# myscale/MyScaleDB

Hardware: NVIDIA H100
Metric: QPS @ recall@10>=0.95 (exact: recall 1.0), FLAT brute-force IP top-10, 10M x 768-d bf16, batch 1024 (higher is better)
Workload: dtype bf16

## Files before the change

### myscaledb_b200/csrc/gemm_common.cuh

```cuda
#pragma once
#include <cuda.h>

#include "common.cuh"
#include "kernels.h"

namespace b200 {
namespace gemm {


constexpr int BM = 128;
constexpr int BN = 256;
constexpr int HN = 128;
constexpr int BK = 64;
constexpr int UMMA_K = 16;
constexpr int EPI_THREADS = 128;
constexpr int NUM_THREADS = EPI_THREADS + 32;
constexpr int SMEM_ALIGN_SLACK = 1024;
constexpr int MAX_STAGES = 4;
constexpr int SMEM_LIMIT = kSmemOptinBytes;

constexpr int SCRATCH_BYTES = 32 * EPI_THREADS * 4;
constexpr int ACC_COLS = 64;
constexpr int ACC_LD = BM + 4;
constexpr int ACC_BYTES = ACC_COLS * ACC_LD * 4;

enum class Operand { BF16, TF32X3, B1 };

template <Operand OP>
struct Layout {
    static constexpr bool F32X3 = OP == Operand::TF32X3;
    static constexpr int KB = F32X3 ? 32 : OP == Operand::B1 ? 128 : 64;
    static constexpr int MMA_K = F32X3 ? 8 : OP == Operand::B1 ? 32 : 16;
    static constexpr int A_PLANE = BM * 128;
    static constexpr int B_PLANE = HN * 128;
    static constexpr int PLANES = F32X3 ? 2 : 1;
    static constexpr int STAGE_BYTES = PLANES * (A_PLANE + B_PLANE);
    static constexpr int TX_BYTES = STAGE_BYTES - (PLANES - 1) * B_PLANE;
    __host__ __device__ static constexpr int off_acc(int st) { return st * STAGE_BYTES; }
    __host__ __device__ static constexpr int off_side(int st) { return off_acc(st) + ACC_BYTES; }
    __host__ __device__ static constexpr int off_bar(int st) { return off_side(st) + 2 * BN * 4; }
    __host__ __device__ static constexpr int off_scratch(int st) { return off_bar(st) + 256; }
    __host__ __device__ static constexpr int off_list(int st) { return off_scratch(st) + SCRATCH_BYTES; }
};

__device__ __forceinline__ void mbar_init(uint64_t *bar, uint32_t count) {
    asm volatile("mbarrier.init.shared::cta.b64 [%0], %1;" ::"r"(smem_u32(bar)), "r"(count));
}
__device__ __forceinline__ void mbar_arrive_expect_tx(uint64_t *bar, uint32_t bytes) {
    asm volatile("mbarrier.arrive.expect_tx.shared::cta.b64 _, [%0], %1;" ::"r"(smem_u32(bar)), "r"(bytes) : "memory");
}
__device__ __forceinline__ void mbar_arrive(uint64_t *bar) {
    asm volatile("mbarrier.arrive.shared::cta.b64 _, [%0];" ::"r"(smem_u32(bar)) : "memory");
}
__device__ __forceinline__ bool mbar_try_wait(uint32_t addr, uint32_t parity) {
    uint32_t ok;
    asm volatile(
        "{\n\t"
        ".reg .pred p;\n\t"
        "mbarrier.try_wait.parity.shared::cta.b64 p, [%1], %2;\n\t"
        "selp.u32 %0, 1, 0, p;\n\t"
        "}\n"
        : "=r"(ok)
        : "r"(addr), "r"(parity)
        : "memory");
    return ok != 0;
}
__device__ __forceinline__ void mbar_wait(uint64_t *bar, uint32_t parity) {
    const uint32_t addr = smem_u32(bar);
    while (!mbar_try_wait(addr, parity)) {
    }
}

__device__ __forceinline__ void tma_load_2d(const CUtensorMap *map, uint64_t *bar, void *dst, int c0, int c1) {
    asm volatile(
        "cp.async.bulk.tensor.2d.shared::cluster.global.mbarrier::complete_tx::bytes [%0], [%1, {%3, %4}], [%2];" ::"r"(
            smem_u32(dst)),
        "l"(reinterpret_cast<uint64_t>(map)), "r"(smem_u32(bar)), "r"(c0), "r"(c1)
        : "memory");
}

__device__ __forceinline__ bool elect_one() {
    uint32_t pred;
    asm volatile(
        "{\n\t"
        ".reg .pred P;\n\t"
        "elect.sync _|P, 0xffffffff;\n\t"
        "selp.b32 %0, 1, 0, P;\n\t"
        "}\n"
        : "=r"(pred));
    return pred != 0;
}

__device__ __forceinline__ uint32_t bound_encode(float f) {
    const uint32_t b = __float_as_uint(f);
    return (b & 0x80000000u) ? ~b : (b | 0x80000000u);
}
__device__ __forceinline__ float bound_decode(uint32_t u) { return (u & 0x80000000u) ? __uint_as_float(u & 0x7fffffffu) : __uint_as_float(~u); }

__device__ __forceinline__ void wg_bar() { asm volatile("bar.sync 1, 128;" ::: "memory"); }

__device__ __forceinline__ uint64_t make_smem_desc(uint32_t smem_addr) {
    uint64_t d = 0;
    d |= (uint64_t)((smem_addr >> 4) & 0x3FFF);
    d |= (uint64_t)1 << 16;
    d |= (uint64_t)(1024 >> 4) << 32;
    d |= (uint64_t)1 << 62;
    return d;
}

__device__ __forceinline__ void wgmma_fence() { asm volatile("wgmma.fence.sync.aligned;" ::: "memory"); }
__device__ __forceinline__ void wgmma_commit() { asm volatile("wgmma.commit_group.sync.aligned;" ::: "memory"); }
template <int N>
__device__ __forceinline__ void wgmma_wait() { asm volatile("wgmma.wait_group.sync.aligned %0;" ::"n"(N) : "memory"); }

#define B200_ACC64_AS(C, v)                                                                                                     \
    C(v[0]), C(v[1]), C(v[2]), C(v[3]), C(v[4]), C(v[5]), C(v[6]), C(v[7]), C(v[8]), C(v[9]), C(v[10]), C(v[11]), C(v[12]),     \
        C(v[13]), C(v[14]), C(v[15]), C(v[16]), C(v[17]), C(v[18]), C(v[19]), C(v[20]), C(v[21]), C(v[22]), C(v[23]), C(v[24]), \
        C(v[25]), C(v[26]), C(v[27]), C(v[28]), C(v[29]), C(v[30]), C(v[31]), C(v[32]), C(v[33]), C(v[34]), C(v[35]), C(v[36]), \
        C(v[37]), C(v[38]), C(v[39]), C(v[40]), C(v[41]), C(v[42]), C(v[43]), C(v[44]), C(v[45]), C(v[46]), C(v[47]), C(v[48]), \
        C(v[49]), C(v[50]), C(v[51]), C(v[52]), C(v[53]), C(v[54]), C(v[55]), C(v[56]), C(v[57]), C(v[58]), C(v[59]), C(v[60]), \
        C(v[61]), C(v[62]), C(v[63])
#define B200_ACC64(v) B200_ACC64_AS("+f", v)
#define B200_ACC64_REGS                                                                                                         \
    "{%0, %1, %2, %3, %4, %5, %6, %7, %8, %9, %10, %11, %12, %13, %14, %15, %16, %17, %18, %19, %20, %21, %22, %23, %24, %25, " \
    "%26, %27, %28, %29, %30, %31, %32, %33, %34, %35, %36, %37, %38, %39, %40, %41, %42, %43, %44, %45, %46, %47, %48, %49, "   \
    "%50, %51, %52, %53, %54, %55, %56, %57, %58, %59, %60, %61, %62, %63}"

__device__ __forceinline__ void wgmma_bf16_n128(float (&d)[64], uint64_t adesc, uint64_t bdesc, uint32_t accum) {
    asm volatile(
        "{\n\t"
        ".reg .pred p;\n\t"
        "setp.ne.b32 p, %66, 0;\n\t"
        "wgmma.mma_async.sync.aligned.m64n128k16.f32.bf16.bf16 " B200_ACC64_REGS ", %64, %65, p, 1, 1, 0, 0;\n\t"
        "}\n"
        : B200_ACC64(d)
        : "l"(adesc), "l"(bdesc), "r"(accum));
}
__device__ __forceinline__ void wgmma_tf32_n128(float (&d)[64], uint64_t adesc, uint64_t bdesc, uint32_t accum) {
    asm volatile(
        "{\n\t"
        ".reg .pred p;\n\t"
        "setp.ne.b32 p, %66, 0;\n\t"
        "wgmma.mma_async.sync.aligned.m64n128k8.f32.tf32.tf32 " B200_ACC64_REGS ", %64, %65, p, 1, 1;\n\t"
        "}\n"
        : B200_ACC64(d)
        : "l"(adesc), "l"(bdesc), "r"(accum));
}
__device__ __forceinline__ void wgmma_b1_n128(int32_t (&d)[64], uint64_t adesc, uint64_t bdesc, uint32_t accum) {
    asm volatile(
        "{\n\t"
        ".reg .pred p;\n\t"
        "setp.ne.b32 p, %66, 0;\n\t"
        "wgmma.mma_async.sync.aligned.m64n128k256.s32.b1.b1.and.popc " B200_ACC64_REGS ", %64, %65, p;\n\t"
        "}\n"
        : B200_ACC64_AS("+r", d)
        : "l"(adesc), "l"(bdesc), "r"(accum));
}

template <int Q, typename T>
__device__ __forceinline__ void acc_store(float *acc, const T (&d0)[64], const T (&d1)[64]) {
    const int warp = (threadIdx.x >> 5) & 3, lane = threadIdx.x & 31;
    const int r = warp * 16 + (lane >> 2), c = 2 * (lane & 3);
#pragma unroll
    for (int j = 0; j < ACC_COLS / 8; j++) {
        const int i = Q * (ACC_COLS / 8) + j;
        float *col = acc + (8 * j + c) * ACC_LD + r;
        col[0] = (float)d0[4 * i];
        col[ACC_LD] = (float)d0[4 * i + 1];
        col[8] = (float)d0[4 * i + 2];
        col[ACC_LD + 8] = (float)d0[4 * i + 3];
        col[64] = (float)d1[4 * i];
        col[ACC_LD + 64] = (float)d1[4 * i + 1];
        col[72] = (float)d1[4 * i + 2];
        col[ACC_LD + 72] = (float)d1[4 * i + 3];
    }
}
__device__ __forceinline__ void acc_load32(const float *acc, int row, int c0, float (&v)[32]) {
    const float *p = acc + c0 * ACC_LD + row;
#pragma unroll
    for (int j = 0; j < 32; j++) v[j] = p[j * ACC_LD];
}

struct ThreadTopK {
    float *keys;
    uint32_t *ids;
    int k, n, worst;
    int tourn;
    float thr_key;
    uint32_t thr_id;
};

__device__ __forceinline__ void list_bind(ThreadTopK &t, float *keys_base, uint32_t *ids_base, int row, int k) {
    t.k = k;
    t.tourn = k >= list_tourn_min_k ? 1 : 0;
    t.keys = keys_base + row;
    t.ids = ids_base + row;
}

__device__ __forceinline__ void list_insert(ThreadTopK &t, float key, uint32_t id) {
    if (!better(key, id, t.thr_key, t.thr_id)) return;
    if (t.tourn) {
        const int G = list_tourn_group(t.k);
        const int ng = (t.k + G - 1) / G;
        if (t.n < t.k) {
            t.keys[t.n * EPI_THREADS] = key;
            t.ids[t.n * EPI_THREADS] = id;
            t.n++;
            if (t.n < t.k) return;
            for (int g = 0; g < ng; g++) {
                const int base = g * G, end = base + G < t.k ? base + G : t.k;
                float wk = t.keys[base * EPI_THREADS];
                uint32_t wi = t.ids[base * EPI_THREADS];
                for (int j = base + 1; j < end; j++) {
                    const float kj = t.keys[j * EPI_THREADS];
                    const uint32_t ij = t.ids[j * EPI_THREADS];
                    if (better(wk, wi, kj, ij)) {
                        wk = kj;
                        wi = ij;
                    }
                }
                t.keys[(t.k + g) * EPI_THREADS] = wk;
                t.ids[(t.k + g) * EPI_THREADS] = wi;
            }
        } else {
            const int g = t.worst;
            const int base = g * G, end = base + G < t.k ? base + G : t.k;
            float wk = 0.f;
            uint32_t wi = 0;
            int slot = -1;
            bool have = false;
            for (int j = base; j < end; j++) {
                float kj = t.keys[j * EPI_THREADS];
                uint32_t ij = t.ids[j * EPI_THREADS];
                if (slot < 0 && kj == t.thr_key && ij == t.thr_id) {
                    slot = j;
                    kj = key;
                    ij = id;
                }
                if (!have || better(wk, wi, kj, ij)) {
                    wk = kj;
                    wi = ij;
                    have = true;
                }
            }
            if (slot < 0) slot = base;
            t.keys[slot * EPI_THREADS] = key;
            t.ids[slot * EPI_THREADS] = id;
            t.keys[(t.k + g) * EPI_THREADS] = wk;
            t.ids[(t.k + g) * EPI_THREADS] = wi;
        }
        float wk = t.keys[t.k * EPI_THREADS];
        uint32_t wi = t.ids[t.k * EPI_THREADS];
        int wg = 0;
        for (int g = 1; g < ng; g++) {
            const float kg = t.keys[(t.k + g) * EPI_THREADS];
            const uint32_t ig = t.ids[(t.k + g) * EPI_THREADS];
            if (better(wk, wi, kg, ig)) {
                wk = kg;
                wi = ig;
                wg = g;
            }
        }
        t.worst = wg;
        t.thr_key = wk;
        t.thr_id = wi;
        return;
    }
    if (t.n < t.k) {
        t.keys[t.n * EPI_THREADS] = key;
        t.ids[t.n * EPI_THREADS] = id;
        t.n++;
        if (t.n < t.k) return;
    } else {
        t.keys[t.worst * EPI_THREADS] = key;
        t.ids[t.worst * EPI_THREADS] = id;
    }
    float wk = t.keys[0];
    uint32_t wi = t.ids[0];
    int wp = 0;
    for (int j = 1; j < t.k; j++) {
        const float kj = t.keys[j * EPI_THREADS];
        const uint32_t ij = t.ids[j * EPI_THREADS];
        if (better(wk, wi, kj, ij)) {
            wk = kj;
            wi = ij;
            wp = j;
        }
    }
    t.worst = wp;
    t.thr_key = wk;
    t.thr_id = wi;
}

static __device__ __noinline__ void list_publish(ThreadTopK &t, float *out_keys, uint32_t *out_ids) {
    for (int i = 1; i < t.n; i++) {
        const float ki = t.keys[i * EPI_THREADS];
        const uint32_t ii = t.ids[i * EPI_THREADS];
        int j = i;
        while (j > 0 && better(ki, ii, t.keys[(j - 1) * EPI_THREADS], t.ids[(j - 1) * EPI_THREADS])) {
            t.keys[j * EPI_THREADS] = t.keys[(j - 1) * EPI_THREADS];
            t.ids[j * EPI_THREADS] = t.ids[(j - 1) * EPI_THREADS];
            j--;
        }
        t.keys[j * EPI_THREADS] = ki;
        t.ids[j * EPI_THREADS] = ii;
    }
    for (int j = 0; j < t.k; j++) {
        out_keys[j] = j < t.n ? t.keys[j * EPI_THREADS] : FLT_MAX;
        out_ids[j] = j < t.n ? t.ids[j * EPI_THREADS] : kNoId;
    }
}

__device__ __forceinline__ void side_fma32(float (&v)[32], const float *scale, const float *bias) {
    const uint32_t sa = smem_u32(scale), ba = smem_u32(bias);
#pragma unroll
    for (int j = 0; j < 32; j += 4) {
        float s0, s1, s2, s3, b0, b1, b2, b3;
        asm volatile("ld.shared.v4.f32 {%0, %1, %2, %3}, [%4];" : "=f"(s0), "=f"(s1), "=f"(s2), "=f"(s3) : "r"(sa + j * 4));
        asm volatile("ld.shared.v4.f32 {%0, %1, %2, %3}, [%4];" : "=f"(b0), "=f"(b1), "=f"(b2), "=f"(b3) : "r"(ba + j * 4));
        v[j] = fmaf(v[j], s0, b0);
        v[j + 1] = fmaf(v[j + 1], s1, b1);
        v[j + 2] = fmaf(v[j + 2], s2, b2);
        v[j + 3] = fmaf(v[j + 3], s3, b3);
    }
}

__device__ __forceinline__ float jaccard_negkey(float v, int pq, float scale, float popc_y) {
    const bool live = scale != 0.f;
    const int x_and = (int)v, x_or = pq + (live ? (int)popc_y : 0) - x_and;
    const float key = x_or == 0 ? 0.f : (float)(x_or - x_and) / (float)x_or;
    return live ? -key : __int_as_float(0xff800000);
}

__device__ __forceinline__ void jaccard_keys32(float (&v)[32], int pq, const float *scale, const float *popc_y) {
    const uint32_t sa = smem_u32(scale), ba = smem_u32(popc_y);
#pragma unroll
    for (int j = 0; j < 32; j += 4) {
        float s[4], b[4];
        asm volatile("ld.shared.v4.f32 {%0, %1, %2, %3}, [%4];" : "=f"(s[0]), "=f"(s[1]), "=f"(s[2]), "=f"(s[3]) : "r"(sa + j * 4));
        asm volatile("ld.shared.v4.f32 {%0, %1, %2, %3}, [%4];" : "=f"(b[0]), "=f"(b[1]), "=f"(b[2]), "=f"(b[3]) : "r"(ba + j * 4));
#pragma unroll
        for (int i = 0; i < 4; i++) v[j + i] = jaccard_negkey(v[j + i], pq, s[i], b[i]);
    }
}

template <int LD = EPI_THREADS>
__device__ __forceinline__ void epilogue_chunk(ThreadTopK &list, float (&v)[32], bool use_side, const float *scale,
                                               const float *bias, uint32_t id0, bool tail, int64_t n, float *scratch,
                                               float ext_bound = FLT_MAX ) {
    const float thr = fminf(list.thr_key, ext_bound);
    bool mine;
    if (use_side) {
        side_fma32(v, scale, bias);
        float m0 = fminf(v[0], v[1]), m1 = fminf(v[2], v[3]), m2 = fminf(v[4], v[5]), m3 = fminf(v[6], v[7]);
#pragma unroll
        for (int j = 8; j < 32; j += 8) {
            m0 = fminf(m0, fminf(v[j], v[j + 1]));
            m1 = fminf(m1, fminf(v[j + 2], v[j + 3]));
            m2 = fminf(m2, fminf(v[j + 4], v[j + 5]));
            m3 = fminf(m3, fminf(v[j + 6], v[j + 7]));
        }
        mine = fminf(fminf(m0, m1), fminf(m2, m3)) <= thr;
    } else {
        float m0 = fmaxf(v[0], v[1]), m1 = fmaxf(v[2], v[3]), m2 = fmaxf(v[4], v[5]), m3 = fmaxf(v[6], v[7]);
#pragma unroll
        for (int j = 8; j < 32; j += 8) {
            m0 = fmaxf(m0, fmaxf(v[j], v[j + 1]));
            m1 = fmaxf(m1, fmaxf(v[j + 2], v[j + 3]));
            m2 = fmaxf(m2, fmaxf(v[j + 4], v[j + 5]));
            m3 = fmaxf(m3, fmaxf(v[j + 6], v[j + 7]));
        }
        mine = fmaxf(fmaxf(m0, m1), fmaxf(m2, m3)) >= -thr;
    }
    if (__any_sync(0xffffffffu, mine)) {
        uint32_t mask = 0;
#pragma unroll
        for (int j = 0; j < 32; j++) {
            const float key = use_side ? v[j] : -v[j];
            scratch[j * LD] = key;
            if (key <= thr) mask |= 1u << j;
        }
        if (tail && !use_side) {
            const int64_t left = n - (int64_t)id0;
            mask = left >= 32 ? mask : left <= 0 ? 0u : (mask & ((1u << left) - 1u));
        }
        while (__any_sync(0xffffffffu, mask != 0)) {
            if (mask) {
                const int j = __ffs(mask) - 1;
                mask &= mask - 1;
                list_insert(list, scratch[j * LD], id0 + (uint32_t)j);
            }
        }
    }
}

typedef CUresult (*EncodeTiledFn)(CUtensorMap *, CUtensorMapDataType, cuuint32_t, void *, const cuuint64_t *,
                                  const cuuint64_t *, const cuuint32_t *, const cuuint32_t *, CUtensorMapInterleave,
                                  CUtensorMapSwizzle, CUtensorMapL2promotion, CUtensorMapFloatOOBfill);

inline EncodeTiledFn get_encode_fn() {
    static EncodeTiledFn fn = nullptr;
    static bool tried = false;
    if (!tried) {
        tried = true;
        void *ptr = nullptr;
        cudaDriverEntryPointQueryResult qres;
        if (cudaGetDriverEntryPoint("cuTensorMapEncodeTiled", &ptr, cudaEnableDefault, &qres) == cudaSuccess &&
            qres == cudaDriverEntryPointSuccess)
            fn = reinterpret_cast<EncodeTiledFn>(ptr);
    }
    return fn;
}

inline bool encode_rows_map(CUtensorMap *map, const void *base, int64_t rows, int d_pad, int box_rows) {
    EncodeTiledFn fn = get_encode_fn();
    if (!fn) return false;
    const cuuint64_t dims[2] = {(cuuint64_t)d_pad, (cuuint64_t)rows};
    const cuuint64_t strides[1] = {(cuuint64_t)d_pad * 2};
    const cuuint32_t box[2] = {(cuuint32_t)BK, (cuuint32_t)box_rows};
    const cuuint32_t estr[2] = {1, 1};
    return fn(map, CU_TENSOR_MAP_DATA_TYPE_BFLOAT16, 2, const_cast<void *>(base), dims, strides, box, estr,
              CU_TENSOR_MAP_INTERLEAVE_NONE, CU_TENSOR_MAP_SWIZZLE_128B, CU_TENSOR_MAP_L2_PROMOTION_L2_256B,
              CU_TENSOR_MAP_FLOAT_OOB_FILL_NONE) == CUDA_SUCCESS;
}

inline bool encode_bytes_map(CUtensorMap *map, const void *base, int64_t rows, int row_bytes, int box_rows) {
    EncodeTiledFn fn = get_encode_fn();
    if (!fn) return false;
    const cuuint64_t dims[2] = {(cuuint64_t)row_bytes, (cuuint64_t)rows};
    const cuuint64_t strides[1] = {(cuuint64_t)row_bytes};
    const cuuint32_t box[2] = {128, (cuuint32_t)box_rows};
    const cuuint32_t estr[2] = {1, 1};
    return fn(map, CU_TENSOR_MAP_DATA_TYPE_UINT8, 2, const_cast<void *>(base), dims, strides, box, estr,
              CU_TENSOR_MAP_INTERLEAVE_NONE, CU_TENSOR_MAP_SWIZZLE_128B, CU_TENSOR_MAP_L2_PROMOTION_L2_256B,
              CU_TENSOR_MAP_FLOAT_OOB_FILL_NONE) == CUDA_SUCCESS;
}

}
}
```

### myscaledb_b200/csrc/ip_gemm_sm90.cu

```cuda
#include <cstdlib>
#include <type_traits>

#include "gemm_common.cuh"

namespace b200 {
namespace gemm {

template <Operand OP>
struct Op {
    using L = Layout<OP>;
    using Acc = typename std::conditional<OP == Operand::B1, int32_t, float>::type;
    static constexpr bool F32X3 = L::F32X3;
    static constexpr int KB = L::KB, MMA_K = L::MMA_K, A_PLANE = L::A_PLANE, B_PLANE = L::B_PLANE, PLANES = L::PLANES;
    static constexpr int WG = gemm_consumer_warpgroups(F32X3);
    static constexpr int THREADS = WG == 1 ? EPI_THREADS + 32 : 3 * EPI_THREADS;
    static constexpr int PRODUCER_REGS = 40, CONSUMER_REGS = 232;
    static constexpr int B_ROWS = WG * HN;
    static constexpr int PASSES = BN / B_ROWS;
    static constexpr int STAGE_BYTES = PLANES * (A_PLANE + WG * B_PLANE);
    static constexpr int TX_BYTES = PLANES * A_PLANE + WG * B_PLANE;
    static constexpr int STAGING_BYTES = 32 * 32 * 4;
    static constexpr int MAX_ST = F32X3 ? 2 : 3;
    static_assert(MAX_ST <= MAX_STAGES, "barrier arrays");
    __host__ __device__ static constexpr int off_staging(int st) { return st * STAGE_BYTES; }
    __host__ __device__ static constexpr int off_bar(int st) { return off_staging(st) + WG * 4 * STAGING_BYTES; }
    __host__ __device__ static constexpr int off_list(int st) { return off_bar(st) + 256; }
    static constexpr int list_bytes(int k_smem) { return k_smem * EPI_THREADS * 8; }
    static size_t smem_bytes(int st, int k_smem) { return (size_t)off_list(st) + (size_t)WG * list_bytes(k_smem) + SMEM_ALIGN_SLACK; }
    static bool lists_fit(int k_smem) { return smem_bytes(2, k_smem) <= (size_t)SMEM_LIMIT; }
    static int stages_for(int k_smem) {
        int st = MAX_ST;
        while (st > 2 && smem_bytes(st, k_smem) > (size_t)SMEM_LIMIT) st--;
        return st;
    }
};

template <int N>
__device__ __forceinline__ void setmaxnreg_inc() { asm volatile("setmaxnreg.inc.sync.aligned.u32 %0;" ::"n"(N)); }
template <int N>
__device__ __forceinline__ void setmaxnreg_dec() { asm volatile("setmaxnreg.dec.sync.aligned.u32 %0;" ::"n"(N)); }

__device__ __forceinline__ void wg_bar(int wg) { asm volatile("bar.sync %0, 128;" ::"r"(wg + 1) : "memory"); }

__device__ __forceinline__ int slot_row(int warp, int slot) { return (slot < 16 ? 0 : 48) + 16 * warp + slot; }

__device__ __forceinline__ float acc_f32(float x) { return x; }
__device__ __forceinline__ float acc_f32(int32_t x) { return __int_as_float(x); }
template <int G, typename T>
__device__ __forceinline__ void group_keys(float (&u)[32], const T (&d0)[64], const T (&d1)[64], bool side, float sc, float bi, int lane) {
#pragma unroll
    for (int i = 0; i < 4; i++) {
        const int x = 4 * (4 * G + i);
        u[2 * i] = acc_f32(d0[x]);
        u[2 * i + 1] = acc_f32(d0[x + 1]);
        u[8 + 2 * i] = acc_f32(d0[x + 2]);
        u[8 + 2 * i + 1] = acc_f32(d0[x + 3]);
        u[16 + 2 * i] = acc_f32(d1[x]);
        u[16 + 2 * i + 1] = acc_f32(d1[x + 1]);
        u[24 + 2 * i] = acc_f32(d1[x + 2]);
        u[24 + 2 * i + 1] = acc_f32(d1[x + 3]);
    }
    if (!side) return;
#pragma unroll
    for (int j = 0; j < 8; j++) {
        const int col = 8 * (j >> 1) + 2 * (lane & 3) + (j & 1);
        const float s = __shfl_sync(0xffffffffu, sc, col), b = __shfl_sync(0xffffffffu, bi, col);
#pragma unroll
        for (int rho = 0; rho < 4; rho++) {
            float &x = u[8 * rho + j];
            x = -fmaf(x, s, b);
        }
    }
}

template <int G = 0, typename T>
__device__ __forceinline__ void group_keys_at(int g, float (&u)[32], const T (&d0)[64], const T (&d1)[64], bool side, const float (&sc)[4],
                                              const float (&bi)[4], int lane) {
    if (g == G) group_keys<G>(u, d0, d1, side, sc[G], bi[G], lane);
    else if constexpr (G + 1 < HN / 32) group_keys_at<G + 1>(g, u, d0, d1, side, sc, bi, lane);
}

__device__ __forceinline__ float quad_rows_max(const float (&m)[4], int lane) {
    const bool b0 = lane & 1, b1 = lane & 2;
    const float s0 = __shfl_xor_sync(0xffffffffu, b0 ? m[0] : m[2], 1);
    const float s1 = __shfl_xor_sync(0xffffffffu, b0 ? m[1] : m[3], 1);
    const float k0 = fmaxf(b0 ? m[2] : m[0], s0), k1 = fmaxf(b0 ? m[3] : m[1], s1);
    const float s = __shfl_xor_sync(0xffffffffu, b1 ? k0 : k1, 2);
    return fmaxf(b1 ? k1 : k0, s);
}

__device__ __forceinline__ void split_tf32(uint32_t x, uint32_t &hi, uint32_t &lo) {
    hi = x & 0xffffe000u;
    const float r = __uint_as_float(x) - __uint_as_float(hi);
    asm("cvt.rna.tf32.f32 %0, %1;" : "=r"(lo) : "f"(r));
}

__global__ void split_tf32_kernel(const float *__restrict__ src, int64_t n_src, int d_pad, float *__restrict__ hi,
                                  float *__restrict__ lo, int64_t n_pad) {
    const int64_t total = n_pad * d_pad;
    for (int64_t i = (int64_t)blockIdx.x * blockDim.x + threadIdx.x; i < total; i += (int64_t)gridDim.x * blockDim.x) {
        const int64_t r = i / d_pad;
        uint32_t h = 0, l = 0;
        if (r < n_src) split_tf32(__float_as_uint(src[i]), h, l);
        hi[i] = __uint_as_float(h);
        lo[i] = __uint_as_float(l);
    }
}

template <Operand OP>
__global__ void __launch_bounds__(Op<OP>::THREADS, 1)
gemm_topk_kernel(const __grid_constant__ CUtensorMap map_q, const __grid_constant__ CUtensorMap map_qlo,
                 const __grid_constant__ CUtensorMap map_c, const GemmTopkParams p) {
    using O = Op<OP>;
    const int STAGES = p.stages;
    extern __shared__ unsigned char smem_dyn[];
    unsigned char *smem = smem_dyn + ((1024u - (smem_u32(smem_dyn) & 1023u)) & 1023u);
    uint64_t *full_bar = reinterpret_cast<uint64_t *>(smem + O::off_bar(STAGES));
    uint64_t *empty_bar = full_bar + MAX_STAGES;

    const int warp = threadIdx.x >> 5, lane = threadIdx.x & 31;
    const int qt = blockIdx.x % p.q_tiles;
    const int worker = blockIdx.x / p.q_tiles;
    const int W = gridDim.x / p.q_tiles;
    const int64_t n_tiles = (p.n + BN - 1) / BN;
    const int kb_count = (p.d_pad + O::KB - 1) / O::KB;

    if (warp == O::WG * 4 && lane == 0) {
        asm volatile("prefetch.tensormap [%0];" ::"l"(reinterpret_cast<uint64_t>(&map_q)) : "memory");
        asm volatile("prefetch.tensormap [%0];" ::"l"(reinterpret_cast<uint64_t>(&map_c)) : "memory");
        for (int i = 0; i < STAGES; i++) {
            mbar_init(&full_bar[i], 1);
            mbar_init(&empty_bar[i], O::WG * 4);
        }
        asm volatile("fence.mbarrier_init.release.cluster;" ::: "memory");
    }
    __syncthreads();

    if (warp >= O::WG * 4) {
        if constexpr (O::WG == 2) setmaxnreg_dec<O::PRODUCER_REGS>();
        if (warp != O::WG * 4) return;
        int stage = 0;
        uint32_t phase = 0;
        int ordinal = 0;
        bool pacing = p.progress != nullptr;
        for (int64_t t = worker; t < n_tiles; t += W, ordinal++) {
            if (pacing) {
                volatile int *prog = p.progress + (size_t)worker * p.q_tiles;
                if (lane == 0) prog[qt] = ordinal + 1;
                __syncwarp();
                int spins = 0;
                while (spins < 256) {
                    bool behind = false;
                    for (int g = lane; g < p.q_tiles; g += 32) behind |= prog[g] < ordinal + 1 - p.sync_slack;
                    if (!__any_sync(0xffffffffu, behind)) break;
                    __nanosleep(200);
                    spins++;
                }
                if (spins >= 256) {
                    if (lane == 0) prog[qt] = 0x7fffffff;
                    pacing = false;
                }
            }
            __syncwarp();
            for (int h = 0; h < O::PASSES; h++) {
                for (int kb = 0; kb < kb_count; kb++) {
                    mbar_wait(&empty_bar[stage], phase ^ 1);
                    if (elect_one()) {
                        unsigned char *st = smem + stage * O::STAGE_BYTES;
                        mbar_arrive_expect_tx(&full_bar[stage], O::TX_BYTES);
                        tma_load_2d(&map_q, &full_bar[stage], st, kb * O::KB, qt * BM);
                        if constexpr (O::F32X3) tma_load_2d(&map_qlo, &full_bar[stage], st + O::A_PLANE, kb * O::KB, qt * BM);
                        tma_load_2d(&map_c, &full_bar[stage], st + O::PLANES * O::A_PLANE, kb * O::KB, (int)(t * BN + h * O::B_ROWS));
                    }
                    __syncwarp();
                    if (++stage == STAGES) {
                        stage = 0;
                        phase ^= 1;
                    }
                }
            }
        }
    } else {
        if constexpr (O::WG == 2) setmaxnreg_inc<O::CONSUMER_REGS>();
        const int wg = threadIdx.x / EPI_THREADS;
        const int tid = threadIdx.x % EPI_THREADS;
        const int wwarp = tid >> 5;
        const int qrow = slot_row(wwarp, lane);
        const bool use_side = p.row_scale || p.row_bias || p.alive || p.scale_const != -1.f;
        const bool jaccard = OP == Operand::B1 && p.jaccard;
        float *staging = reinterpret_cast<float *>(smem + O::off_staging(STAGES) + (wg * 4 + wwarp) * O::STAGING_BYTES);
        const uint32_t staging_s = smem_u32(staging);
        const size_t producer = ((size_t)worker * O::WG + wg) * p.q_tiles + qt;
        ThreadTopK list;
        list.n = 0;
        list.worst = 0;
        list.thr_key = (qt * BM + qrow < p.nq_valid) ? FLT_MAX : -FLT_MAX;
        list.thr_id = 0;
        const int list_cap = list_cap_for(p.k);
        if (p.lists_in_smem) {
            unsigned char *lists = smem + O::off_list(STAGES) + wg * O::list_bytes(list_cap);
            list_bind(list, reinterpret_cast<float *>(lists), reinterpret_cast<uint32_t *>(lists + O::list_bytes(list_cap) / 2), tid, p.k);
        } else {
            list_bind(list, p.list_keys_gmem + producer * list_cap * EPI_THREADS, p.list_ids_gmem + producer * list_cap * EPI_THREADS,
                      tid, p.k);
        }
        const int q = qt * BM + qrow;
        const bool live = q < p.nq_valid;
        const int pq = (jaccard && live) ? (int)p.q_popc[q] : 0;
        const uint32_t smem0 = smem_u32(smem);
        int stage = 0;
        uint32_t phase = 0;
        typename O::Acc d0[64], d1[64];
        for (int64_t t = worker; t < n_tiles; t += W) {
            const int64_t n0 = t * BN;
            const bool tail = n0 + BN > p.n;
            for (int pass = 0; pass < O::PASSES; pass++) {
                const int h = O::WG == 1 ? pass : wg;
                const uint32_t bound_u = live ? __ldcg(p.query_bound + q) : 0xffffffffu;
                float sc[HN / 32] = {}, bi[HN / 32] = {};
                if (use_side) {
#pragma unroll
                    for (int g = 0; g < HN / 32; g++) {
                        const int64_t r = n0 + h * HN + 32 * g + lane;
                        bool ok = r < p.n;
                        if (ok && p.alive) ok = (p.alive[r >> 3] >> (r & 7)) & 1;
                        sc[g] = ok ? (p.row_scale ? p.row_scale[r] : p.scale_const) : 0.f;
                        bi[g] = ok ? (p.row_bias ? p.row_bias[r] : 0.f) : __int_as_float(0x7f800000);
                    }
                }
                int prev = -1;
                for (int kb = 0; kb < kb_count; kb++) {
                    mbar_wait(&full_bar[stage], phase);
                    const uint32_t st = smem0 + stage * O::STAGE_BYTES;
                    if constexpr (O::F32X3) {
                        uint4 *b = reinterpret_cast<uint4 *>(smem + stage * O::STAGE_BYTES + 2 * O::A_PLANE);
                        uint4 *bl = b + O::B_PLANE / 16;
#pragma unroll
                        for (int i = 0; i < O::B_PLANE / 16 / EPI_THREADS; i++) {
                            const uint4 raw = b[tid + i * EPI_THREADS];
                            uint4 hi, lo;
                            split_tf32(raw.x, hi.x, lo.x);
                            split_tf32(raw.y, hi.y, lo.y);
                            split_tf32(raw.z, hi.z, lo.z);
                            split_tf32(raw.w, hi.w, lo.w);
                            b[tid + i * EPI_THREADS] = hi;
                            bl[tid + i * EPI_THREADS] = lo;
                        }
                        asm volatile("fence.proxy.async.shared::cta;" ::: "memory");
                        wg_bar(wg);
                    }
                    wgmma_fence();
                    if constexpr (O::F32X3) {
                        const uint64_t ahi = make_smem_desc(st), alo = make_smem_desc(st + O::A_PLANE);
                        const uint64_t b = make_smem_desc(st + 2 * O::A_PLANE), blo = make_smem_desc(st + 2 * O::A_PLANE + O::B_PLANE);
                        constexpr uint64_t M1 = (64 * 128) >> 4;
#pragma unroll
                        for (int k = 0; k < O::KB / O::MMA_K; k++) {
                            const uint64_t off = (uint64_t)(k * (O::MMA_K * 4 >> 4));
                            const uint32_t acc0 = (kb | k) != 0 ? 1u : 0u;
                            wgmma_tf32_n128(d0, alo + off, b + off, acc0);
                            wgmma_tf32_n128(d1, alo + M1 + off, b + off, acc0);
                            wgmma_tf32_n128(d0, ahi + off, blo + off, 1u);
                            wgmma_tf32_n128(d1, ahi + M1 + off, blo + off, 1u);
                            wgmma_tf32_n128(d0, ahi + off, b + off, 1u);
                            wgmma_tf32_n128(d1, ahi + M1 + off, b + off, 1u);
                        }
                    } else if constexpr (OP == Operand::B1) {
                        const uint64_t a = make_smem_desc(st), b = make_smem_desc(st + O::A_PLANE + wg * O::B_PLANE);
                        constexpr uint64_t M1 = (64 * 128) >> 4;
#pragma unroll
                        for (int k = 0; k < O::KB / O::MMA_K; k++) {
                            const uint64_t off = (uint64_t)(k * (O::MMA_K >> 4));
                            const uint32_t acc0 = (kb | k) != 0 ? 1u : 0u;
                            wgmma_b1_n128(d0, a + off, b + off, acc0);
                            wgmma_b1_n128(d1, a + M1 + off, b + off, acc0);
                        }
                    } else {
                        const uint64_t a = make_smem_desc(st), b = make_smem_desc(st + O::A_PLANE + wg * O::B_PLANE);
                        constexpr uint64_t M1 = (64 * 128) >> 4;
#pragma unroll
                        for (int k = 0; k < O::KB / O::MMA_K; k++) {
                            const uint64_t off = (uint64_t)(k * (O::MMA_K * 2 >> 4));
                            const uint32_t acc0 = (kb | k) != 0 ? 1u : 0u;
                            wgmma_bf16_n128(d0, a + off, b + off, acc0);
                            wgmma_bf16_n128(d1, a + M1 + off, b + off, acc0);
                        }
                    }
                    wgmma_commit();
                    wgmma_wait<1>();
                    if (prev >= 0) {
                        __syncwarp();
                        if (lane == 0) mbar_arrive(&empty_bar[prev]);
                    }
                    prev = stage;
                    if (++stage == STAGES) {
                        stage = 0;
                        phase ^= 1;
                    }
                }
                wgmma_wait<0>();
                __syncwarp();
                if (lane == 0) mbar_arrive(&empty_bar[prev]);
                if constexpr (OP == Operand::B1) {
#pragma unroll
                    for (int i = 0; i < 64; i++) {
                        d0[i] = __float_as_int((float)d0[i]);
                        d1[i] = __float_as_int((float)d1[i]);
                    }
                }
                const float bound = bound_u == 0xffffffffu ? FLT_MAX : bound_decode(bound_u);
                const float thr = __shfl_sync(0xffffffffu, fminf(list.thr_key, bound), (lane >> 2) + 8 * (2 * (lane & 1) + ((lane >> 1) & 1)));
                uint32_t slow = jaccard ? (1u << HN / 32) - 1 : 0;
                if (!jaccard) {
#pragma unroll
                    for (int g = 0; g < HN / 32; g++) {
                        float u[32], m[4];
                        group_keys_at(g, u, d0, d1, use_side, sc, bi, lane);
#pragma unroll
                        for (int rho = 0; rho < 4; rho++) {
                            const float *x = u + 8 * rho;
                            m[rho] = fmaxf(fmaxf(fmaxf(x[0], x[1]), fmaxf(x[2], x[3])), fmaxf(fmaxf(x[4], x[5]), fmaxf(x[6], x[7])));
                        }
                        if (__any_sync(0xffffffffu, quad_rows_max(m, lane) >= -thr)) slow |= 1u << g;
                    }
                }
#pragma unroll 1
                while (slow) {
                    const int g = __ffs(slow) - 1;
                    slow &= slow - 1;
                    float u[32];
                    group_keys_at(g, u, d0, d1, use_side && !jaccard, sc, bi, lane);
#pragma unroll
                    for (int j = 0; j < 8; j++) {
                        const int col = 8 * (j >> 1) + 2 * (lane & 3) + (j & 1);
#pragma unroll
                        for (int rho = 0; rho < 4; rho++) {
                            const uint32_t a = staging_s + 4 * (col * 32 + (((lane >> 2) + 8 * rho) ^ (8 * (lane & 3))));
                            asm volatile("st.shared.f32 [%0], %1;" ::"r"(a), "f"(u[8 * rho + j]) : "memory");
                        }
                    }
                    __syncwarp();
                    float v[32];
#pragma unroll
                    for (int j = 0; j < 32; j++) {
                        const uint32_t a = staging_s + 4 * (j * 32 + (lane ^ (8 * ((j >> 1) & 3))));
                        asm volatile("ld.shared.f32 %0, [%1];" : "=f"(v[j]) : "r"(a) : "memory");
                    }
                    __syncwarp();
                    if (jaccard) {
                        const float s = g == 0 ? sc[0] : g == 1 ? sc[1] : g == 2 ? sc[2] : sc[3];
                        const float b = g == 0 ? bi[0] : g == 1 ? bi[1] : g == 2 ? bi[2] : bi[3];
#pragma unroll
                        for (int j = 0; j < 32; j++) v[j] = jaccard_negkey(v[j], pq, __shfl_sync(0xffffffffu, s, j), __shfl_sync(0xffffffffu, b, j));
                    }
                    epilogue_chunk<32>(list, v, false, nullptr, nullptr, (uint32_t)(n0 + h * HN + 32 * g), tail, p.n, staging + lane,
                                       bound);
                    __syncwarp();
                }
                if (live && list.n == list.k && list.thr_key < bound && fabsf(list.thr_key) <= FLT_MAX)
                    atomicMin(p.query_bound + q, bound_encode(list.thr_key));
            }
        }
        float *ok = p.part_keys + (producer * BM + qrow) * p.k;
        uint32_t *oi = p.part_ids + (producer * BM + qrow) * p.k;
        list_publish(list, ok, oi);
    }
}

static bool encode_map(CUtensorMap *map, const void *base, int64_t rows, int d_pad, int box_rows, Operand op) {
    EncodeTiledFn fn = get_encode_fn();
    if (!fn) return false;
    const int es = op == Operand::TF32X3 ? 4 : op == Operand::BF16 ? 2 : 1;
    const CUtensorMapDataType type = op == Operand::TF32X3 ? CU_TENSOR_MAP_DATA_TYPE_FLOAT32
                                     : op == Operand::BF16 ? CU_TENSOR_MAP_DATA_TYPE_BFLOAT16
                                                           : CU_TENSOR_MAP_DATA_TYPE_UINT8;
    const cuuint64_t dims[2] = {(cuuint64_t)d_pad, (cuuint64_t)rows};
    const cuuint64_t strides[1] = {(cuuint64_t)d_pad * es};
    const cuuint32_t box[2] = {(cuuint32_t)(128 / es), (cuuint32_t)box_rows};
    const cuuint32_t estr[2] = {1, 1};
    return fn(map, type, 2, const_cast<void *>(base), dims, strides, box, estr, CU_TENSOR_MAP_INTERLEAVE_NONE,
              CU_TENSOR_MAP_SWIZZLE_128B, CU_TENSOR_MAP_L2_PROMOTION_L2_256B, CU_TENSOR_MAP_FLOAT_OOB_FILL_NONE) == CUDA_SUCCESS;
}

template <Operand OP>
static cudaError_t launch(const CUtensorMap &map_q, const CUtensorMap &map_qlo, const CUtensorMap &map_c, const GemmTopkParams &p_in,
                          int grid, cudaStream_t s) {
    using O = Op<OP>;
    GemmTopkParams p = p_in;
    const int list_cap = list_cap_for(p.k);
    p.lists_in_smem = O::lists_fit(list_cap) ? 1 : 0;
    const int k_smem = p.lists_in_smem ? list_cap : 0;
    p.stages = O::stages_for(k_smem);
    const size_t smem = O::smem_bytes(p.stages, k_smem);
    auto kern = gemm_topk_kernel<OP>;
    cudaError_t e = cudaFuncSetAttribute(kern, cudaFuncAttributeMaxDynamicSharedMemorySize, (int)smem);
    if (e != cudaSuccess) return e;
    kern<<<grid, O::THREADS, smem, s>>>(map_q, map_qlo, map_c, p);
    g_launches++;
    return cudaGetLastError();
}

}

int gemm_topk_grid(int q_tiles, int64_t n, int num_sms) {
    const int64_t n_tiles = ceil_div(n, gemm::BN);
    int64_t g = (int64_t)q_tiles * (n_tiles < 1 ? 1 : n_tiles);
    if (g > num_sms) g = num_sms;
    if (g < q_tiles) g = q_tiles;
    return (int)g;
}

cudaError_t launch_split_tf32(const float *src, int64_t n_src, int d_pad, float *hi, float *lo, int64_t n_pad, cudaStream_t s) {
    if (n_pad == 0) return cudaSuccess;
    int64_t b = ceil_div(n_pad * d_pad, 256);
    if (b > 132 * 8) b = 132 * 8;
    gemm::split_tf32_kernel<<<(int)b, 256, 0, s>>>(src, n_src, d_pad, hi, lo, n_pad);
    g_launches++;
    return cudaGetLastError();
}

cudaError_t launch_gemm_topk(const GemmTopkParams &p, int grid, cudaStream_t s, const char **err_detail) {
    *err_detail = nullptr;
    if (grid % p.q_tiles != 0) {
        *err_detail = "grid must be a multiple of q_tiles";
        return cudaErrorInvalidValue;
    }
    CUtensorMap map_q, map_c;
    if (!gemm::encode_map(&map_q, p.queries_bf16, p.nq_pad, p.d_pad, gemm::BM, gemm::Operand::BF16) ||
        !gemm::encode_map(&map_c, p.corpus_bf16, p.n, p.d_pad, gemm::Op<gemm::Operand::BF16>::B_ROWS, gemm::Operand::BF16)) {
        *err_detail = "cuTensorMapEncodeTiled failed";
        return cudaErrorInvalidValue;
    }
    return gemm::launch<gemm::Operand::BF16>(map_q, map_q, map_c, p, grid, s);
}

cudaError_t launch_gemm3_topk(const GemmTopkParams &p, int grid, cudaStream_t s, const char **err_detail) {
    *err_detail = nullptr;
    if (grid % p.q_tiles != 0 || !p.queries_lo) {
        *err_detail = "gemm3: grid must be a multiple of q_tiles, queries_lo set";
        return cudaErrorInvalidValue;
    }
    CUtensorMap map_qhi, map_qlo, map_c;
    if (!gemm::encode_map(&map_qhi, p.queries_bf16, p.nq_pad, p.d_pad, gemm::BM, gemm::Operand::TF32X3) ||
        !gemm::encode_map(&map_qlo, p.queries_lo, p.nq_pad, p.d_pad, gemm::BM, gemm::Operand::TF32X3) ||
        !gemm::encode_map(&map_c, p.corpus_bf16, p.n, p.d_pad, gemm::Op<gemm::Operand::TF32X3>::B_ROWS, gemm::Operand::TF32X3)) {
        *err_detail = "cuTensorMapEncodeTiled failed";
        return cudaErrorInvalidValue;
    }
    return gemm::launch<gemm::Operand::TF32X3>(map_qhi, map_qlo, map_c, p, grid, s);
}

cudaError_t launch_gemm_b1_topk(const GemmTopkParams &p, int grid, cudaStream_t s, const char **err_detail) {
    *err_detail = nullptr;
    if (grid % p.q_tiles != 0 || p.d_pad % 16 != 0 || !p.row_bias || (p.jaccard && !p.q_popc)) {
        *err_detail = "gemm b1: grid must be a multiple of q_tiles, rows a multiple of 16 bytes, popcounts set";
        return cudaErrorInvalidValue;
    }
    CUtensorMap map_q, map_c;
    if (!gemm::encode_map(&map_q, p.queries_bf16, p.nq_pad, p.d_pad, gemm::BM, gemm::Operand::B1) ||
        !gemm::encode_map(&map_c, p.corpus_bf16, p.n, p.d_pad, gemm::Op<gemm::Operand::B1>::B_ROWS, gemm::Operand::B1)) {
        *err_detail = "cuTensorMapEncodeTiled failed";
        return cudaErrorInvalidValue;
    }
    return gemm::launch<gemm::Operand::B1>(map_q, map_q, map_c, p, grid, s);
}

}
```

Before: 40790.

## Use m64n256 wgmma with per-warpgroup M split for two-warpgroup configs

When two consumer warpgroups are present, each warpgroup now owns 64 query rows and issues one m64n256 wgmma covering the full 256-column tile, instead of each taking a 128-column half with two m64n128 calls. This halves the number of wgmma instructions and lets a single descriptor pair cover both column halves, cutting issue overhead and reloads of the same B tile. The epilogue remaps rows and columns (slot_row, col_half), folds Jaccard scaling into group_keys, and adds a half-tile path at the tail that zeroes d1. The extra code paths and index remapping add risk, and the producer-partition indexing changes.

```diff
diff --git a/myscaledb_b200/csrc/gemm_common.cuh b/myscaledb_b200/csrc/gemm_common.cuh
--- a/myscaledb_b200/csrc/gemm_common.cuh
+++ b/myscaledb_b200/csrc/gemm_common.cuh
@@ -154,6 +154,35 @@
         "wgmma.mma_async.sync.aligned.m64n128k256.s32.b1.b1.and.popc " B200_ACC64_REGS ", %64, %65, p;\n\t"
         "}\n"
         : B200_ACC64_AS("+r", d)
+        : "l"(adesc), "l"(bdesc), "r"(accum));
+}
+
+#define B200_ACC128_REGS                                                                                                        \
+    "{%0, %1, %2, %3, %4, %5, %6, %7, %8, %9, %10, %11, %12, %13, %14, %15, %16, %17, %18, %19, %20, %21, %22, %23, %24, "     \
+    "%25, %26, %27, %28, %29, %30, %31, %32, %33, %34, %35, %36, %37, %38, %39, %40, %41, %42, %43, %44, %45, %46, %47, %48, " \
+    "%49, %50, %51, %52, %53, %54, %55, %56, %57, %58, %59, %60, %61, %62, %63, %64, %65, %66, %67, %68, %69, %70, %71, %72, " \
+    "%73, %74, %75, %76, %77, %78, %79, %80, %81, %82, %83, %84, %85, %86, %87, %88, %89, %90, %91, %92, %93, %94, %95, %96, " \
+    "%97, %98, %99, %100, %101, %102, %103, %104, %105, %106, %107, %108, %109, %110, %111, %112, %113, %114, %115, %116, "    \
+    "%117, %118, %119, %120, %121, %122, %123, %124, %125, %126, %127}"
+
+__device__ __forceinline__ void wgmma_bf16_n256(float (&d0)[64], float (&d1)[64], uint64_t adesc, uint64_t bdesc, uint32_t accum) {
+    asm volatile(
+        "{\n\t"
+        ".reg .pred p;\n\t"
+        "setp.ne.b32 p, %130, 0;\n\t"
+        "wgmma.mma_async.sync.aligned.m64n256k16.f32.bf16.bf16 " B200_ACC128_REGS ", %128, %129, p, 1, 1, 0, 0;\n\t"
+        "}\n"
+        : B200_ACC64(d0), B200_ACC64(d1)
+        : "l"(adesc), "l"(bdesc), "r"(accum));
+}
+__device__ __forceinline__ void wgmma_b1_n256(int32_t (&d0)[64], int32_t (&d1)[64], uint64_t adesc, uint64_t bdesc, uint32_t accum) {
+    asm volatile(
+        "{\n\t"
+        ".reg .pred p;\n\t"
+        "setp.ne.b32 p, %130, 0;\n\t"
+        "wgmma.mma_async.sync.aligned.m64n256k256.s32.b1.b1.and.popc " B200_ACC128_REGS ", %128, %129, p;\n\t"
+        "}\n"
+        : B200_ACC64_AS("+r", d0), B200_ACC64_AS("+r", d1)
         : "l"(adesc), "l"(bdesc), "r"(accum));
 }
 
diff --git a/myscaledb_b200/csrc/ip_gemm_sm90.cu b/myscaledb_b200/csrc/ip_gemm_sm90.cu
--- a/myscaledb_b200/csrc/ip_gemm_sm90.cu
+++ b/myscaledb_b200/csrc/ip_gemm_sm90.cu
@@ -15,6 +15,7 @@
     static constexpr int WG = gemm_consumer_warpgroups(F32X3);
     static constexpr int THREADS = WG == 1 ? EPI_THREADS + 32 : 3 * EPI_THREADS;
     static constexpr int PRODUCER_REGS = 40, CONSUMER_REGS = 232;
+    static constexpr bool N256 = WG == 2;
     static constexpr int B_ROWS = WG * HN;
     static constexpr int PASSES = BN / B_ROWS;
     static constexpr int STAGE_BYTES = PLANES * (A_PLANE + WG * B_PLANE);
@@ -42,12 +43,17 @@
 
 __device__ __forceinline__ void wg_bar(int wg) { asm volatile("bar.sync %0, 128;" ::"r"(wg + 1) : "memory"); }
 
-__device__ __forceinline__ int slot_row(int warp, int slot) { return (slot < 16 ? 0 : 48) + 16 * warp + slot; }
+template <bool N256>
+__device__ __forceinline__ int slot_row(int wg, int warp, int slot) {
+    return N256 ? 64 * wg + 16 * warp + (slot & 15) : (slot < 16 ? 0 : 48) + 16 * warp + slot;
+}
 
 __device__ __forceinline__ float acc_f32(float x) { return x; }
 __device__ __forceinline__ float acc_f32(int32_t x) { return __int_as_float(x); }
-template <int G, typename T>
-__device__ __forceinline__ void group_keys(float (&u)[32], const T (&d0)[64], const T (&d1)[64], bool side, float sc, float bi, int lane) {
+template <int G, bool N256, typename T>
+__device__ __forceinline__ void group_keys(float (&u)[32], const T (&d0)[64], const T (&d1)[64], bool side,
+                                           const float (&sc)[N256 ? 8 : 4], const float (&bi)[N256 ? 8 : 4], int lane,
+                                           bool jaccard, int pq_r, int pq_r8) {
 #pragma unroll
     for (int i = 0; i < 4; i++) {
         const int x = 4 * (4 * G + i);
@@ -64,20 +70,27 @@
 #pragma unroll
     for (int j = 0; j < 8; j++) {
         const int col = 8 * (j >> 1) + 2 * (lane & 3) + (j & 1);
-        const float s = __shfl_sync(0xffffffffu, sc, col), b = __shfl_sync(0xffffffffu, bi, col);
+        const float s0 = __shfl_sync(0xffffffffu, sc[G], col), b0 = __shfl_sync(0xffffffffu, bi[G], col);
+        float s1 = s0, b1 = b0;
+        if constexpr (N256) {
+            s1 = __shfl_sync(0xffffffffu, sc[G + HN / 32], col);
+            b1 = __shfl_sync(0xffffffffu, bi[G + HN / 32], col);
+        }
 #pragma unroll
         for (int rho = 0; rho < 4; rho++) {
             float &x = u[8 * rho + j];
-            x = -fmaf(x, s, b);
-        }
-    }
-}
-
-template <int G = 0, typename T>
-__device__ __forceinline__ void group_keys_at(int g, float (&u)[32], const T (&d0)[64], const T (&d1)[64], bool side, const float (&sc)[4],
-                                              const float (&bi)[4], int lane) {
-    if (g == G) group_keys<G>(u, d0, d1, side, sc[G], bi[G], lane);
-    else if constexpr (G + 1 < HN / 32) group_keys_at<G + 1>(g, u, d0, d1, side, sc, bi, lane);
+            x = jaccard ? jaccard_negkey(x, rho & 1 ? pq_r8 : pq_r, rho < 2 ? s0 : s1, rho < 2 ? b0 : b1)
+                        : -fmaf(x, rho < 2 ? s0 : s1, rho < 2 ? b0 : b1);
+        }
+    }
+}
+
+template <bool N256, int G = 0, typename T>
+__device__ __forceinline__ void group_keys_at(int g, float (&u)[32], const T (&d0)[64], const T (&d1)[64], bool side,
+                                              const float (&sc)[N256 ? 8 : 4], const float (&bi)[N256 ? 8 : 4], int lane,
+                                              bool jaccard = false, int pq_r = 0, int pq_r8 = 0) {
+    if (g == G) group_keys<G, N256>(u, d0, d1, side, sc, bi, lane, jaccard, pq_r, pq_r8);
+    else if constexpr (G + 1 < HN / 32) group_keys_at<N256, G + 1>(g, u, d0, d1, side, sc, bi, lane, jaccard, pq_r, pq_r8);
 }
 
 __device__ __forceinline__ float quad_rows_max(const float (&m)[4], int lane) {
@@ -185,12 +198,12 @@
         const int wg = threadIdx.x / EPI_THREADS;
         const int tid = threadIdx.x % EPI_THREADS;
         const int wwarp = tid >> 5;
-        const int qrow = slot_row(wwarp, lane);
+        const int qrow = slot_row<O::N256>(wg, wwarp, lane);
+        const int col_half = O::N256 ? lane >> 4 : 0;
         const bool use_side = p.row_scale || p.row_bias || p.alive || p.scale_const != -1.f;
         const bool jaccard = OP == Operand::B1 && p.jaccard;
         float *staging = reinterpret_cast<float *>(smem + O::off_staging(STAGES) + (wg * 4 + wwarp) * O::STAGING_BYTES);
         const uint32_t staging_s = smem_u32(staging);
-        const size_t producer = ((size_t)worker * O::WG + wg) * p.q_tiles + qt;
         ThreadTopK list;
         list.n = 0;
         list.worst = 0;
@@ -201,12 +214,14 @@
             unsigned char *lists = smem + O::off_list(STAGES) + wg * O::list_bytes(list_cap);
             list_bind(list, reinterpret_cast<float *>(lists), reinterpret_cast<uint32_t *>(lists + O::list_bytes(list_cap) / 2), tid, p.k);
         } else {
-            list_bind(list, p.list_keys_gmem + producer * list_cap * EPI_THREADS, p.list_ids_gmem + producer * list_cap * EPI_THREADS,
+            const size_t region = ((size_t)worker * O::WG + wg) * p.q_tiles + qt;
+            list_bind(list, p.list_keys_gmem + region * list_cap * EPI_THREADS, p.list_ids_gmem + region * list_cap * EPI_THREADS,
                       tid, p.k);
         }
         const int q = qt * BM + qrow;
         const bool live = q < p.nq_valid;
         const int pq = (jaccard && live) ? (int)p.q_popc[q] : 0;
+        const int pq_r = __shfl_sync(0xffffffffu, pq, lane >> 2), pq_r8 = __shfl_sync(0xffffffffu, pq, (lane >> 2) + 8);
         const uint32_t smem0 = smem_u32(smem);
         int stage = 0;
         uint32_t phase = 0;
@@ -215,13 +230,14 @@
             const int64_t n0 = t * BN;
             const bool tail = n0 + BN > p.n;
             for (int pass = 0; pass < O::PASSES; pass++) {
-                const int h = O::WG == 1 ? pass : wg;
+                const int64_t c0 = n0 + pass * O::B_ROWS;
+                const bool half_tile = O::N256 && c0 + HN >= p.n;
                 const uint32_t bound_u = live ? __ldcg(p.query_bound + q) : 0xffffffffu;
-                float sc[HN / 32] = {}, bi[HN / 32] = {};
+                float sc[O::B_ROWS / 32] = {}, bi[O::B_ROWS / 32] = {};
                 if (use_side) {
 #pragma unroll
-                    for (int g = 0; g < HN / 32; g++) {
-                        const int64_t r = n0 + h * HN + 32 * g + lane;
+                    for (int g = 0; g < O::B_ROWS / 32; g++) {
+                        const int64_t r = c0 + 32 * g + lane;
                         bool ok = r < p.n;
                         if (ok && p.alive) ok = (p.alive[r >> 3] >> (r & 7)) & 1;
                         sc[g] = ok ? (p.row_scale ? p.row_scale[r] : p.scale_const) : 0.f;
@@ -265,25 +281,20 @@
                             wgmma_tf32_n128(d0, ahi + off, b + off, 1u);
                             wgmma_tf32_n128(d1, ahi + M1 + off, b + off, 1u);
                         }
-                    } else if constexpr (OP == Operand::B1) {
-                        const uint64_t a = make_smem_desc(st), b = make_smem_desc(st + O::A_PLANE + wg * O::B_PLANE);
-                        constexpr uint64_t M1 = (64 * 128) >> 4;
+                    } else {
+                        const uint64_t a = make_smem_desc(st + wg * (64 * 128)), b = make_smem_desc(st + O::A_PLANE);
 #pragma unroll
                         for (int k = 0; k < O::KB / O::MMA_K; k++) {
-                            const uint64_t off = (uint64_t)(k * (O::MMA_K >> 4));
                             const uint32_t acc0 = (kb | k) != 0 ? 1u : 0u;
-                            wgmma_b1_n128(d0, a + off, b + off, acc0);
-                            wgmma_b1_n128(d1, a + M1 + off, b + off, acc0);
-                        }
-                    } else {
-                        const uint64_t a = make_smem_desc(st), b = make_smem_desc(st + O::A_PLANE + wg * O::B_PLANE);
-                        constexpr uint64_t M1 = (64 * 128) >> 4;
-#pragma unroll
-                        for (int k = 0; k < O::KB / O::MMA_K; k++) {
-                            const uint64_t off = (uint64_t)(k * (O::MMA_K * 2 >> 4));
-                            const uint32_t acc0 = (kb | k) != 0 ? 1u : 0u;
-                            wgmma_bf16_n128(d0, a + off, b + off, acc0);
-                            wgmma_bf16_n128(d1, a + M1 + off, b + off, acc0);
+                            if constexpr (OP == Operand::B1) {
+                                const uint64_t off = (uint64_t)(k * (O::MMA_K >> 4));
+                                if (half_tile) wgmma_b1_n128(d0, a + off, b + off, acc0);
+                                else wgmma_b1_n256(d0, d1, a + off, b + off, acc0);
+                            } else {
+                                const uint64_t off = (uint64_t)(k * (O::MMA_K * 2 >> 4));
+                                if (half_tile) wgmma_bf16_n128(d0, a + off, b + off, acc0);
+                                else wgmma_bf16_n256(d0, d1, a + off, b + off, acc0);
+                            }
                         }
                     }
                     wgmma_commit();
@@ -301,6 +312,10 @@
                 wgmma_wait<0>();
                 __syncwarp();
                 if (lane == 0) mbar_arrive(&empty_bar[prev]);
+                if (half_tile) {
+#pragma unroll
+                    for (int i = 0; i < 64; i++) d1[i] = 0;
+                }
                 if constexpr (OP == Operand::B1) {
 #pragma unroll
                     for (int i = 0; i < 64; i++) {
@@ -315,7 +330,7 @@
 #pragma unroll
                     for (int g = 0; g < HN / 32; g++) {
                         float u[32], m[4];
-                        group_keys_at(g, u, d0, d1, use_side, sc, bi, lane);
+                        group_keys_at<O::N256>(g, u, d0, d1, use_side, sc, bi, lane);
 #pragma unroll
                         for (int rho = 0; rho < 4; rho++) {
                             const float *x = u + 8 * rho;
@@ -329,7 +344,7 @@
                     const int g = __ffs(slow) - 1;
                     slow &= slow - 1;
                     float u[32];
-                    group_keys_at(g, u, d0, d1, use_side && !jaccard, sc, bi, lane);
+                    group_keys_at<O::N256>(g, u, d0, d1, use_side, sc, bi, lane, jaccard, pq_r, pq_r8);
 #pragma unroll
                     for (int j = 0; j < 8; j++) {
                         const int col = 8 * (j >> 1) + 2 * (lane & 3) + (j & 1);
@@ -347,20 +362,15 @@
                         asm volatile("ld.shared.f32 %0, [%1];" : "=f"(v[j]) : "r"(a) : "memory");
                     }
                     __syncwarp();
-                    if (jaccard) {
-                        const float s = g == 0 ? sc[0] : g == 1 ? sc[1] : g == 2 ? sc[2] : sc[3];
-                        const float b = g == 0 ? bi[0] : g == 1 ? bi[1] : g == 2 ? bi[2] : bi[3];
-#pragma unroll
-                        for (int j = 0; j < 32; j++) v[j] = jaccard_negkey(v[j], pq, __shfl_sync(0xffffffffu, s, j), __shfl_sync(0xffffffffu, b, j));
-                    }
-                    epilogue_chunk<32>(list, v, false, nullptr, nullptr, (uint32_t)(n0 + h * HN + 32 * g), tail, p.n, staging + lane,
-                                       bound);
+                    epilogue_chunk<32>(list, v, false, nullptr, nullptr, (uint32_t)(c0 + HN * col_half + 32 * g), tail, p.n,
+                                       staging + lane, bound);
                     __syncwarp();
                 }
                 if (live && list.n == list.k && list.thr_key < bound && fabsf(list.thr_key) <= FLT_MAX)
                     atomicMin(p.query_bound + q, bound_encode(list.thr_key));
             }
         }
+        const size_t producer = ((size_t)worker * O::WG + col_half) * p.q_tiles + qt;
         float *ok = p.part_keys + (producer * BM + qrow) * p.k;
         uint32_t *oi = p.part_ids + (producer * BM + qrow) * p.k;
         list_publish(list, ok, oi);
```

Result: slower. 38690, median of 6 (-5.1%).
